# mjsargent/gym-miniworld

Measured on AMD Instinct MI355X. Metric: env-steps/s (80x60 RGB obs), higher is better.
Workload: dtype f64 sim / f32 render / u8 obs; 1 GPU; maze8192; env_id=MiniWorld-Maze-v0, envs_per_gpu=8192, global_envs=8192, obs=80x60 RGB, domain_rand=False, actions=uniform random over {turn_left, turn_right, move_forward}, counter-based, auto_reset=True, parallelism=env-sharded x1

## Files before the change

### gym_miniworld_amd/build.py

```python
import os
import subprocess
import sys

HERE = os.path.dirname(os.path.abspath(__file__))
CSRC = os.path.join(HERE, "csrc")
SOURCES = ["mwb_api.hip", "mwb_kernels.hip", "mwb_copy.hip", "mwb_repeat.hip", "mwb_rollout.hip"]
HEADERS = ["mwb_internal.h", "mwb_task_table.h", "mwb_copy_check.h", "mwb_repeat_fold.h", "mwb_rollout_map.h", "mwb_dispatch_map.h", "mwb_lds_layout.h", "mwb_glibc_trig.h", "mwb_sincos_table.inc", "mwb_texture_host.h", os.path.join("..", "..", "include", "miniworld_batch.h")]
OUT = os.path.join(HERE, "libmwbatch.so")
REMARKS = os.path.join(HERE, "libmwbatch.resources.txt")
FLAGS = ["--offload-arch=gfx950", "-O3", "-std=c++17", "-fPIC", "-shared", "-ffp-contract=off", "-Wall",
         "-Wno-unused-value"]


def needs_build():
    if not os.path.exists(OUT):
        return True
    t = os.path.getmtime(OUT)
    return any(os.path.getmtime(os.path.join(CSRC, f)) > t for f in SOURCES + HEADERS)


def source_digest():
    import hashlib
    h = hashlib.sha1()
    for f in SOURCES + HEADERS:
        with open(os.path.join(CSRC, f), "rb") as fh:
            h.update(fh.read())
    h.update(" ".join(FLAGS).encode())
    return h.hexdigest()


# ... 27 lines not shown
```

### gym_miniworld_amd/csrc/mwb_api.hip

```cpp
#include <math.h>
#include <stdio.h>
#include <stdlib.h>
#include <string.h>

#include <string>
#include <type_traits>
#include <vector>

#include "mwb_internal.h"
#include "mwb_lds_layout.h"
#include "mwb_rollout_map.h"
#include "mwb_task_table.h"
#include "mwb_texture_host.h"

static_assert(mwb_task_frame_words(1) == MWB_FRAME_WORDS_FOR(1) && mwb_task_frame_words(MWB_MAX_ENTS) == MWB_FRAME_WORDS_FOR(MWB_MAX_ENTS),
              "mwb_task_table.h restates the frame constants' size");

static thread_local std::string g_err;
static int set_err(int code, const std::string &msg) { g_err = msg; return code; }
#define HIP_TRY(expr)                                                                       \
    do {                                                                                    \
        hipError_t _e = (expr);                                                             \
        if (_e != hipSuccess)                                                               \
            return set_err(MWB_EHIP, std::string(#expr) + ": " + hipGetErrorString(_e));    \
// ... 200 lines not shown
    {
        std::string why;
        if (int rc = mwb_resolve_task(*cfg, &t, &why)) return set_err(rc, why);
    }

    mwb_handle *h = new mwb_handle();
    h->cfg = *cfg;
    h->serial = g_next_serial++;
    MwbDev &d = h->dev;
    d.N = cfg->num_envs; d.task = cfg->task; d.W = cfg->obs_width; d.H = cfg->obs_height;
    d.want_depth = cfg->want_depth ? 1 : 0; d.layout = cfg->layout; d.domain_rand = cfg->domain_rand ? 1 : 0;
    d.auto_reset = cfg->no_auto_reset ? 0 : 1;
    d.ent_task = t.ent_task; d.n_boxes = t.n_boxes; d.R_max = t.R_max; d.S_max = t.S_max; d.max_episode_steps = t.max_episode_steps;
    d.n_tex = t.n_tex; d.no_ceiling = t.no_ceiling; d.poly = t.poly; d.room_words = t.room_words; d.frame_words = t.frame_words;
    d.agent_radius = t.agent_radius;
    memcpy(d.task_args, t.task_args, sizeof(d.task_args));
    double P[MWB_NPARAM][9];
    if (cfg->use_default_params) default_params(P); else memcpy(P, cfg->params, sizeof(P));
    for (int i = 0; i < MWB_NPARAM; i++)
        for (int k = 0; k < 3; k++) { d.params[i].def[k] = P[i][k]; d.params[i].lo[k] = P[i][3 + k]; d.params[i].hi[k] = P[i][6 + k]; }
    d.stk_cpf = 3;
    { const char *dbg = getenv("MWB_DEBUG"); d.debug_flags = dbg ? atoi(dbg) : 0; }
    { const char *ex = getenv("MWB_EXP"); d.exp_flags = ex ? atoi(ex) : 0; }
    { const char *no = getenv("MWB_NO_OVERLAP"); h->overlap_reset = !(no && atoi(no)); }
    {
        const char *sp = getenv("MWB_SPLIT");
        int split = sp ? atoi(sp) : 768;
        d.split_envs = split < 0 ? 0 : (split > cfg->num_envs ? cfg->num_envs : split);
    }
    if (d.ent_task) {
        int tw_ = 0, th_ = 0;
        const char *tl = getenv("MWB_TILE");
        if (tl && sscanf(tl, "%dx%d", &tw_, &th_) != 2) { tw_ = 0; th_ = 0; }
        if (tw_ > 0 && th_ > 0) { d.tile_w = tw_ < d.W ? tw_ : d.W; d.tile_h = th_ < d.H ? th_ : d.H; }
    }
    if (d.tile_w == 0 && (mwb_render_lds_bytes(d) > 160 * 1024 || !mwb_pixel_queue_fits(d.W, d.H))) {
        int tw = 0, th = 0;
        mwb_view_tile(&tw, &th);
        d.tile_w = tw < d.W ? tw : d.W; d.tile_h = th < d.H ? th : d.H;
    }
    { const char *no = getenv("MWB_NO_FRAME_REUSE"); h->frame_reuse = !(no && atoi(no)) && d.tile_w == 0; }

    const size_t N = (size_t)d.N;
    int rc = MWB_OK;
    mwb_for_each_env_array(d, d, h->frame_reuse, [&](auto *&, auto *&p, const MwbEnvArray &a) {
        if (rc == MWB_OK) rc = dev_alloc(h, &p, mwb_env_array_elems(a, N));
// ... 728 lines not shown
    if (render) { rc = ensure_ready(dst); if (rc) return rc; }
    hipStream_t s = (hipStream_t)stream;
    MwbDev &d = dst->dev;
    if (!dst->copy_dst_pairs) { rc = dev_alloc(dst, &dst->copy_dst_pairs, (size_t)d.N); if (rc) return rc; }
    if (!dst->copy_src_mark) { rc = dev_alloc(dst, &dst->copy_src_mark, (size_t)d.N); if (rc) return rc; }
    if (!dst->copy_rejected) {
        rc = dev_alloc(dst, &dst->copy_rejected, (size_t)1); if (rc) return rc;
        HIP_TRY(hipDeviceSynchronize());
    }
    if (dst->copy_pairs_cap < (size_t)count) {
        if (dst->copy_pairs) { HIP_TRY(hipFree(dst->copy_pairs)); dst->copy_pairs = nullptr; dst->copy_pairs_cap = 0; }
        const size_t cap = (size_t)count < (size_t)d.N ? (size_t)d.N : (size_t)count;
        HIP_TRY(hipMalloc((void **)&dst->copy_pairs, cap * sizeof(int2)));
        dst->copy_pairs_cap = cap;
    }
    const int slot = copy_table_for(dst, src);
    if (slot < 0) return slot;
    const mwb_handle::CopyTable &tab = dst->copy_table[slot];
    mwb_launch_copy_validate(dst_idx_dev, src_idx_dev, count, d.N, src->dev.N, same ? 1 : 0, dst->copy_dst_pairs, dst->copy_src_mark,
                             dst->copy_pairs, dst->copy_rejected, s);
    rc = check_launch("copy_validate_kernel"); if (rc) return rc;
    mwb_launch_copy_envs(dst->copy_tables + (size_t)slot * MWB_COPY_TABLE_DESCS, tab.n_small, tab.small_chunks, tab.n_large, dst->copy_pairs, count, s);
    rc = check_launch("copy_envs_kernel"); if (rc) return rc;
    dst->have_world = true;
    if (render) {
        d.step_pass = 0; d.reuse_pass = 0;
        dst->timing_now = false;
        mwb_launch_copy_list(d, dst->copy_pairs, count, 0, s);
        rc = check_launch("copy_list_kernel"); if (rc) return rc;
        mwb_launch_prep(d, 1, s);
        rc = check_launch("prep_kernel"); if (rc) return rc;
        mwb_launch_render(d, 1, s);
        rc = check_launch("render_kernel"); if (rc) return rc;
        mwb_launch_copy_list(d, dst->copy_pairs, count, 1, s);
        rc = check_launch("copy_list_kernel"); if (rc) return rc;
    } else {
        mwb_launch_copy_list(d, dst->copy_pairs, count, 2, s);
        rc = check_launch("copy_list_kernel"); if (rc) return rc;
    }
    if (copy_window) {
        const size_t plane = (size_t)d.W * d.H * (dst->stack_dtype == 1 ? 4 : 1), C = (size_t)dst->stack_n * dst->stack_cpf;
        const size_t kd = dst->stack_planes ? (size_t)dst->stack_planes : C, ks = src->stack_planes ? (size_t)src->stack_planes : C;
        const size_t pd = dst->stack_planes ? (size_t)dst->stack_pos : 0, ps = src->stack_planes ? (size_t)src->stack_pos : 0;
        mwb_launch_copy_stack((char *)dst->stack, kd * plane, pd * plane, (const char *)src->stack, ks * plane, ps * plane, C * plane, dst->copy_pairs, count, s);
        rc = check_launch("copy_stack_kernel"); if (rc) return rc;
    }
// ... 390 lines not shown
```

### gym_miniworld_amd/csrc/mwb_copy.hip

```cpp
#include "mwb_internal.h"
#include "mwb_copy_check.h"

#define COPY_THREADS 256

__global__ void __launch_bounds__(COPY_THREADS) copy_validate_kernel(int phase, const int32_t *__restrict__ dst_idx, const int32_t *__restrict__ src_idx,
                                                                     int count, int n_dst, int n_src, int same_handle, int32_t *__restrict__ dst_pairs,
                                                                     uint8_t *__restrict__ src_mark, int2 *__restrict__ pairs,
                                                                     unsigned long long *__restrict__ rejected) {
    for (size_t i = (size_t)blockIdx.x * COPY_THREADS + threadIdx.x; i < (size_t)count; i += (size_t)gridDim.x * COPY_THREADS) {
        const int32_t dst = dst_idx[i], src = src_idx[i];
        if (phase == 0) {
            if (mwb_copy_counts_dst(dst, n_dst)) atomicAdd(dst_pairs + dst, 1);
            if (mwb_copy_marks_src(dst, src, n_src, same_handle)) src_mark[src] = 1;
        } else if (phase == 1) {
            const bool in = mwb_copy_index_ok(dst, n_dst);
            const int v = mwb_copy_verdict(dst, src, n_dst, n_src, same_handle, in ? dst_pairs[dst] : 0, in && same_handle ? src_mark[dst] : 0);
            pairs[i] = v == MWB_PAIR_COPY ? make_int2(dst, src) : make_int2(-1, -1);
            if (v == MWB_PAIR_REJECTED) atomicAdd(rejected, 1ull);
        } else {
            if (mwb_copy_counts_dst(dst, n_dst)) dst_pairs[dst] = 0;
            if (mwb_copy_marks_src(dst, src, n_src, same_handle)) src_mark[src] = 0;
        }
    }
}
// ... 34 lines not shown
            if (wide) for (uint32_t b = 0; b < t.elem; b += 8) *(uint64_t *)(d + b) = *(const uint64_t *)(s + b);
            else for (uint32_t b = 0; b < t.elem; b += 4) *(uint32_t *)(d + b) = *(const uint32_t *)(s + b);
        }
    }
}

__global__ void __launch_bounds__(COPY_THREADS) copy_list_kernel(MwbDev d, const int2 *__restrict__ pairs, int count, int what) {
    if (what == 1 && blockIdx.x == 0 && threadIdx.x == 0) d.reset_count[0] = 0;
    for (size_t i = (size_t)blockIdx.x * COPY_THREADS + threadIdx.x; i < (size_t)count; i += (size_t)gridDim.x * COPY_THREADS) {
        const int dst = pairs[i].x;
        if (dst < 0) continue;
        if (what == 0) {
            d.reset_set[dst] = 1;
            const int at = atomicAdd(d.reset_count, 1);
            if (at < d.N) d.reset_list[at] = dst;
        } else if (what == 1) {
            d.reset_set[dst] = 0;
        } else if (d.frame_cached) {
            d.frame_cached[dst] = 0;
        }
    }
}

#define COPY_STACK_RUN 32768
__global__ void __launch_bounds__(COPY_THREADS) copy_stack_kernel(char *dst, size_t env_bytes_dst, size_t off_dst, const char *src,
                                                                  size_t env_bytes_src, size_t off_src, size_t window_bytes, const int2 *__restrict__ pairs) {
    const int2 p = pairs[blockIdx.x];
    if (p.x < 0) return;
    const size_t b0 = (size_t)blockIdx.y * COPY_STACK_RUN, n = window_bytes - b0 < COPY_STACK_RUN ? window_bytes - b0 : COPY_STACK_RUN;
    copy_run(dst + (size_t)p.x * env_bytes_dst + off_dst + b0, src + (size_t)p.y * env_bytes_src + off_src + b0, n);
}

static inline unsigned pair_blocks(int count) {
    const long long b = ((long long)count + COPY_THREADS - 1) / COPY_THREADS;
    return (unsigned)(b < 1 ? 1 : b > 4096 ? 4096 : b);
}

void mwb_launch_copy_validate(const int32_t *dst_idx, const int32_t *src_idx, int count, int n_dst, int n_src, int same_handle,
                              int32_t *dst_pairs, uint8_t *src_mark, int2 *pairs, unsigned long long *rejected, hipStream_t s) {
    for (int phase = 0; phase < 3; phase++)
        hipLaunchKernelGGL(copy_validate_kernel, dim3(pair_blocks(count)), dim3(COPY_THREADS), 0, s, phase, dst_idx, src_idx, count, n_dst, n_src,
                           same_handle, dst_pairs, src_mark, pairs, rejected);
}

void mwb_launch_copy_envs(const MwbCopyDesc *table, int n_small, int small_chunks, int n_large, const int2 *pairs, int count, hipStream_t s) {
    if (n_small > 0 && small_chunks > 0)
        hipLaunchKernelGGL(copy_envs_kernel<false>, dim3((unsigned)small_chunks, pair_blocks(count)), dim3(COPY_THREADS), 0, s, table, n_small, pairs, count);
    if (n_large > 0)
        hipLaunchKernelGGL(copy_envs_kernel<true>, dim3((unsigned)count, (unsigned)n_large), dim3(COPY_THREADS), 0, s, table, n_small, pairs, count);
}

void mwb_launch_copy_list(const MwbDev &d, const int2 *pairs, int count, int what, hipStream_t s) {
    hipLaunchKernelGGL(copy_list_kernel, dim3(pair_blocks(count)), dim3(COPY_THREADS), 0, s, d, pairs, count, what);
}

void mwb_launch_copy_stack(char *dst, size_t env_bytes_dst, size_t off_dst, const char *src, size_t env_bytes_src, size_t off_src,
                           size_t window_bytes, const int2 *pairs, int count, hipStream_t s) {
    const unsigned runs = (unsigned)((window_bytes + COPY_STACK_RUN - 1) / COPY_STACK_RUN);
    hipLaunchKernelGGL(copy_stack_kernel, dim3((unsigned)count, runs), dim3(COPY_THREADS), 0, s, dst, env_bytes_dst, off_dst, src, env_bytes_src,
                       off_src, window_bytes, pairs);
}
```

### gym_miniworld_amd/csrc/mwb_internal.h

```cpp
#pragma once
#include <hip/hip_runtime.h>
#include <stdint.h>

#include "../../include/miniworld_batch.h"

#define MWB_MT_WORDS 625
#define MWB_MAX_TEX MWB_NUM_TEXTURES
#define MWB_MAX_LEVELS 12
#define MWB_MAX_BOXES 6
#define MWB_RESET_MAX_BLOCKS 4096
#define MWB_ENT_AGENT 255
#define MWB_ORDER_STRIDE 24

#define RW_MINX 0
#define RW_MAXX 1
#define RW_MINZ 2
#define RW_MAXZ 3
#define RW_HEIGHT 4
#define RW_TEX 5
#define RW_NBR01 6
#define RW_NBR23 7
#define RW_SIDE0 8
#define RW_SIDE_WORDS 4
#define RS_LO 0
#define RS_HI 1
#define RS_MAXY 2
#define RS_UORG 3
// ... 132 lines not shown
    int32_t *n_order;
    double *task_f;
    int32_t *task_i;
    int32_t *text_tex;
    int32_t *ovr_slot;
    double *ovr_pose;
    const MwbMeshDesc *mesh_desc;
    const float4 *mesh_data;
    MwbMeshDims mesh_dims[MWB_MAX_MESH_DIMS];
    int n_mesh_dims;
    uint8_t *frame_cache;
    float *depth_cache;
    uint8_t *frame_cached;
    uint8_t *frame_same;
    int reuse_pass;
    unsigned long long *reuse_stats;
    int tile_w, tile_h;
    unsigned long long *dbg_counters;
    int exp_flags;
    int32_t *render_list;
    int32_t *reuse_list;
    int32_t *list_counts;
    const uint8_t *frozen;
};

struct MwbEnvArray {
    const char *name;
    bool minor;
    uint32_t rows;
    size_t per;
    const char *not_copied;
};
static inline size_t mwb_env_array_elems(const MwbEnvArray &a, size_t N) { return N * a.rows * a.per; }

template <class Dev, class F>
static inline void mwb_for_each_env_array(Dev &s, Dev &d, bool frame_reuse, F &&f) {
#define MWB_MINOR(p, rows, per, when, why) if (when) f(s.p, d.p, MwbEnvArray{#p, true, (uint32_t)(rows), (size_t)(per), why})
#define MWB_MAJOR(p, count, when, why) if (when) f(s.p, d.p, MwbEnvArray{#p, false, 1u, (size_t)(count), why})
    const char *const COPIED = nullptr;
    const char *const OUTPUT = "an output of the last transition or render: the next one rewrites it";
    const char *const DISPATCH = "dispatch scratch: a heuristic or a work list rebuilt before every launch";
    const char *const CACHE = "the copy pass and the render it runs maintain the cached frames and their flags";
    const int B = s.n_boxes;
    const bool always = true, ent = s.ent_task != 0, depth = s.want_depth != 0;
    const size_t pixels = (size_t)s.W * s.H;
    MWB_MINOR(agent_x, 1, 1, always, COPIED); MWB_MINOR(agent_z, 1, 1, always, COPIED); MWB_MINOR(agent_dir, 1, 1, always, COPIED);
    MWB_MINOR(box_x, B, 1, always, COPIED); MWB_MINOR(box_z, B, 1, always, COPIED); MWB_MINOR(box_dir, B, 1, always, COPIED);
    MWB_MINOR(box_y, B, 1, always, COPIED); MWB_MINOR(box_color, B, 3, always, COPIED); MWB_MINOR(box_size, B, 1, always, COPIED);
    MWB_MINOR(carrying, 1, 1, always, COPIED); MWB_MINOR(goal_dist, 1, 1, always, COPIED);
    MWB_MINOR(episode_count, 1, 1, always, COPIED); MWB_MINOR(task_step_count, 1, 1, always, COPIED); MWB_MINOR(goal_idx, 1, 1, always, COPIED);
    MWB_MAJOR(cam, 4, always, COPIED); MWB_MAJOR(sky_color, 3, always, COPIED); MWB_MAJOR(light_pos, 3, always, COPIED);
    MWB_MAJOR(light_color, 3, always, COPIED); MWB_MAJOR(light_ambient, 3, always, COPIED);
    MWB_MINOR(step_count, 1, 1, always, COPIED); MWB_MINOR(n_rooms, 1, 1, always, COPIED); MWB_MINOR(n_segs, 1, 1, always, COPIED);
    MWB_MINOR(n_rrooms, 1, 1, always, COPIED);
    MWB_MAJOR(world_ext, 4, always, COPIED);
    MWB_MAJOR(rng, MWB_MT_WORDS, always, COPIED);
    MWB_MAJOR(rooms, (size_t)s.R_max * s.room_words, always, COPIED);
    MWB_MINOR(segs, s.S_max * 4, 1, always, COPIED);
    MWB_MINOR(ent_meta, B, 1, ent, COPIED); MWB_MINOR(ent_radius, B, 1, ent, COPIED); MWB_MINOR(ent_height, B, 1, ent, COPIED);
    MWB_MINOR(ent_scale, B, 1, ent, COPIED);
    MWB_MAJOR(ent_order, MWB_ORDER_STRIDE, ent, COPIED); MWB_MINOR(n_order, 1, 1, ent, COPIED);
    MWB_MINOR(task_f, 1, 1, ent, COPIED); MWB_MINOR(task_i, 1, 1, ent, COPIED); MWB_MAJOR(text_tex, 8, ent, COPIED);
    MWB_MINOR(ovr_slot, 1, 1, ent, COPIED); MWB_MAJOR(ovr_pose, 4, ent, COPIED);
    MWB_MAJOR(frame, s.frame_words, always, "prep_kernel rebuilds it before every render");
    MWB_MINOR(reset_set, 1, 1, always, "the copy pass sets and clears it around the render it runs");
    MWB_MINOR(reset_list, 1, 1, always, "the copy pass sets and clears it around the render it runs");
    MWB_MAJOR(obs, pixels * 3, always, OUTPUT); MWB_MAJOR(depth, pixels, depth, OUTPUT);
    MWB_MAJOR(cost, 2, always, DISPATCH); MWB_MINOR(bucket, 1, 1, always, DISPATCH);
    MWB_MINOR(order_bufs[0], 1, 1, always, DISPATCH); MWB_MINOR(order_bufs[1], 1, 1, always, DISPATCH);
    MWB_MINOR(render_list, 1, 1, always, DISPATCH); MWB_MINOR(reuse_list, 1, 1, always, DISPATCH);
    MWB_MAJOR(frame_cache, pixels * 3, frame_reuse, CACHE); MWB_MAJOR(depth_cache, pixels, frame_reuse && depth, CACHE);
    MWB_MINOR(frame_cached, 1, 1, frame_reuse, CACHE); MWB_MINOR(frame_same, 1, 1, frame_reuse, CACHE);
#undef MWB_MINOR
#undef MWB_MAJOR
}

struct MwbCopyDesc {
    const char *src;
    char *dst;
    uint32_t rows, elem;
    uint64_t src_stride, dst_stride;
    uint32_t first_chunk;
    uint32_t pad;
};
#define MWB_COPY_SMALL_ELEM 32
#define MWB_COPY_ROW_CHUNK 8

template <class F>
static inline void mwb_for_each_copied_array(const MwbDev &s, const MwbDev &d, F &&f) {
    mwb_for_each_env_array(s, d, false, [&](auto *sp, auto *dp, const MwbEnvArray &a) {
        if (a.not_copied) return;
        const uint64_t elem = sizeof(*sp) * a.per;
        f((const char *)sp, (char *)dp, a.rows, (uint32_t)elem, a.minor ? elem * (uint64_t)s.N : 0, a.minor ? elem * (uint64_t)d.N : 0);
    });
}

void mwb_launch_copy_validate(const int32_t *dst_idx, const int32_t *src_idx, int count, int n_dst, int n_src, int same_handle,
                              int32_t *dst_pairs, uint8_t *src_mark, int2 *pairs, unsigned long long *rejected, hipStream_t s);
void mwb_launch_copy_envs(const MwbCopyDesc *table, int n_small, int small_chunks, int n_large, const int2 *pairs, int count, hipStream_t s);
void mwb_launch_copy_list(const MwbDev &d, const int2 *pairs, int count, int what, hipStream_t s);
void mwb_launch_copy_stack(char *dst, size_t env_bytes_dst, size_t off_dst, const char *src, size_t env_bytes_src, size_t off_src,
                           size_t window_bytes, const int2 *pairs, int count, hipStream_t s);

void mwb_launch_repeat_fold(const MwbDev &d, int sub, int last, int repeat, const uint8_t *skip, const int32_t *counts, double *sum,
                            int32_t *taken, uint8_t *same, uint8_t *frozen, hipStream_t s);

struct MwbRollout {
    int N, T, nstack, R;
    int grey;
    int base, cursor;
    size_t frame_bytes;
    char *ring;
    uint8_t *age;
    float *reward, *mask, *feature;
    unsigned long long *rejected;
};
void mwb_launch_rollout_push(const MwbRollout &r, int t, int after_reset, const uint8_t *fresh_dev, const uint8_t *done, const float *reward,
                             const float *feature, hipStream_t s);
void mwb_launch_rollout_after_update(const MwbRollout &r, hipStream_t s);
void mwb_launch_rollout_gather(const MwbRollout &r, const int64_t *index, int count, void *out, int out_float, hipStream_t s);

void mwb_launch_step(const MwbDev &d, const int32_t *actions, const uint8_t *skip_mask, hipStream_t s);
void mwb_launch_clear_list(const MwbDev &d, hipStream_t s);
// ... 18 lines not shown
```

### gym_miniworld_amd/csrc/mwb_kernels.hip

```cpp
#include <type_traits>

#include "mwb_internal.h"
#include "mwb_glibc_trig.h"
#include "mwb_lds_layout.h"
#include "mwb_dispatch_map.h"

__device__ __forceinline__ double ref_sin(double x) { return mwb_trig::in_range(x) ? mwb_trig::sin_glibc(x) : sin(x); }
__device__ __forceinline__ double ref_cos(double x) { return mwb_trig::in_range(x) ? mwb_trig::cos_glibc(x) : cos(x); }

__device__ __forceinline__ uint32_t mt_temper(uint32_t y) {
    y ^= (y >> 11);
    y ^= (y << 7) & 0x9d2c5680u;
    y ^= (y << 15) & 0xefc60000u;
    y ^= (y >> 18);
    return y;
}

__device__ __forceinline__ uint32_t mt_mix(uint32_t a, uint32_t b, uint32_t c) {
    uint32_t y = (a & 0x80000000u) | (b & 0x7fffffffu);
    return c ^ (y >> 1) ^ ((y & 1u) ? 0x9908b0dfu : 0u);
}

struct MtSerial {
    uint32_t *key;
// ... 47 lines not shown
        uint32_t mask = rng;
        mask |= mask >> 1; mask |= mask >> 2; mask |= mask >> 4; mask |= mask >> 8; mask |= mask >> 16;
        uint32_t v;
        do { v = next32() & mask; } while (v > rng);
        return lo + (int)v;
    }
};

template <class SegPtr>
__device__ __forceinline__ bool seg_hit(SegPtr sg, double px, double pz, double radius) {
    double ax = sg[0], az = sg[1], bx = sg[2], bz = sg[3];
    double abx = bx - ax, abz = bz - az;
    double apx = px - ax, apz = pz - az;
    double dotAPAB = (apx * abx + 0.0) + apz * abz;
    double dotABAB = (abx * abx + 0.0) + abz * abz;
    double proj = dotAPAB / dotABAB;
    proj = proj < 0 ? 0 : (proj > 1 ? 1 : proj);
    double cx = ax + proj * abx, cz = az + proj * abz;
    double ddx = cx - px, ddz = cz - pz;
    double dist = sqrt((ddx * ddx + 0.0) + ddz * ddz);
    return dist < radius;
}


__device__ __forceinline__ double tagged_add(double a, bool a_f32, double b, bool b_f32, bool &res_f32) {
    res_f32 = a_f32 || b_f32;
    return res_f32 ? (double)((float)a + (float)b) : a + b;
}
__device__ __forceinline__ double tagged_add(double a, bool a_f32, double b, bool b_f32) { bool f; return tagged_add(a, a_f32, b, b_f32, f); }

__device__ __forceinline__ double box_radius(double size) {
    double sx = size, sz = size;
    return sqrt(sx * sx + sz * sz) / 2;
}

#define STEP_PARTS 8
template <int NBX>
__global__ void __launch_bounds__(64 * STEP_PARTS) step_kernel(MwbDev d, const int32_t *__restrict__ actions,
                                                                const uint8_t *__restrict__ skip) {
    __shared__ double s_nx[64], s_nz[64];
    __shared__ int s_move[64], s_hit[64];
    const int lane = threadIdx.x & 63, part = threadIdx.x >> 6;
    const int e = blockIdx.x * 64 + lane;
    const bool in_range = e < d.N;
    const bool frozen = in_range && d.frozen && d.frozen[e];
    const bool dummy = in_range && !frozen && skip && skip[e];
    const bool live = in_range && !dummy && !frozen;
    int sc = 0, a = -1;
    double ax = 0, az = 0, adir = 0, nx = 0, nz = 0, turn_step = 0;
    constexpr int NB = NBX;
    double bx[NBX], bz[NBX], by[NBX], brad[NBX], bsz[NBX];
#pragma unroll
    for (int b = 0; b < NBX; b++) { bx[b] = 0; bz[b] = 0; by[b] = 0; brad[b] = 0; bsz[b] = 0; }
    int carried = -1;
    bool same = true;
    const double arad = d.agent_radius;
    if (blockIdx.x == 0 && threadIdx.x == 0 && d.order_state[1]) {
        d.order_state[0] ^= 1; d.order_state[1] = 0;
    }
    if (part == 0) {
        s_move[lane] = 0; s_hit[lane] = 0;
        if (dummy) {
            d.reward[e] = -99.0f; d.reward64[e] = -99.0; d.done[e] = 0; d.ep_steps[e] = d.step_count[e];
            d.reset_set[e] = 0;
            d.feature[e * 2] = 0.0f; d.feature[e * 2 + 1] = 0.0f;
            if (d.frame_same) d.frame_same[e] = d.frame_cached[e];
        }
        if (live) {
            a = actions[(size_t)e * d.act_stride];
            if (d.act_stride == 2 && actions[(size_t)e * 2 + 1] != (a >> 31)) a = -1;
            ax = d.agent_x[e]; az = d.agent_z[e]; adir = d.agent_dir[e];
#pragma unroll
            for (int b = 0; b < NBX; b++)
                if (b < NB) {
                    const size_t be = (size_t)b * d.N + e;
                    bx[b] = d.box_x[be]; bz[b] = d.box_z[be]; by[b] = d.box_y[be]; bsz[b] = d.box_size[be]; brad[b] = box_radius(bsz[b]);
                }
            carried = d.carrying[e];
            MtSerial g;
            const bool use_rng = d.domain_rand || d.task == MWB_TASK_SIM2REAL_PUSH;
            if (use_rng) g.load(d.rng + (size_t)e * MWB_MT_WORDS);
// ... 32 lines not shown
                }
            }
            sc = d.step_count[e] + 1;
            d.step_count[e] = sc;
            double fwd_step = d.params[MWB_P_FORWARD_STEP].def[0];
            double fwd_drift = d.params[MWB_P_FORWARD_DRIFT].def[0];
            turn_step = d.params[MWB_P_TURN_STEP].def[0];
            if (d.domain_rand) {
                fwd_step = g.uniform(d.params[MWB_P_FORWARD_STEP].lo[0], d.params[MWB_P_FORWARD_STEP].hi[0]);
                fwd_drift = g.uniform(d.params[MWB_P_FORWARD_DRIFT].lo[0], d.params[MWB_P_FORWARD_DRIFT].hi[0]);
                turn_step = g.uniform(d.params[MWB_P_TURN_STEP].lo[0], d.params[MWB_P_TURN_STEP].hi[0]);
            }
            if (use_rng) g.store();
            if (a == 2 || a == 3) {
                double fd = (a == 2) ? fwd_step : -fwd_step;
                double c = ref_cos(adir), s = ref_sin(adir);
                nx = (ax + c * fd) + s * fwd_drift;
                nz = (az + (-s) * fd) + c * fwd_drift;
                s_nx[lane] = nx; s_nz[lane] = nz; s_move[lane] = 1;
            }
        }
    }
    __syncthreads();
    if (live && s_move[lane]) {
        const double px = s_nx[lane], pz = s_nz[lane];
        const double *sg = d.segs + e;
        const size_t N = (size_t)d.N;
        const int ns = d.n_segs[e];
        bool hit = false;
        const double guard = arad + 1e-9;
        for (int i0 = part * 8; i0 < ns; i0 += 8 * STEP_PARTS) {
            double q[8][4];
#pragma unroll
            for (int k = 0; k < 8; k++) {
                const int i = (i0 + k < ns) ? i0 + k : ns - 1;
#pragma unroll
                for (int c = 0; c < 4; c++) q[k][c] = sg[(size_t)(i * 4 + c) * N];
            }
#pragma unroll
            for (int k = 0; k < 8; k++) {
                bool nearby = px >= fmin(q[k][0], q[k][2]) - guard && px <= fmax(q[k][0], q[k][2]) + guard &&
                              pz >= fmin(q[k][1], q[k][3]) - guard && pz <= fmax(q[k][1], q[k][3]) + guard;
                if (nearby) hit = seg_hit(q[k], px, pz, arad) || hit;
            }
        }
        if (hit) s_hit[lane] = 1;
    }
    __syncthreads();
    if (part != 0 || !live) return;
    const double max_fwd = d.params[MWB_P_FORWARD_STEP].hi[0];
    auto pick = [&](const double (&v)[NBX], int i) {
        double r_ = v[0];
#pragma unroll
        for (int b = 1; b < NBX; b++) r_ = (i == b) ? v[b] : r_;
        return r_;
    };
    auto intersect_serial = [&](int self_idx, double px, double pz, double radius, bool test_walls) {
        if (test_walls) {
            const int ns = d.n_segs[e];
            for (int i = 0; i < ns; i++) {
                double q[4];
#pragma unroll
                for (int c = 0; c < 4; c++) q[c] = d.segs[(size_t)(i * 4 + c) * d.N + e];
                if (seg_hit(q, px, pz, radius)) return 1;
            }
        }
        int res = 0;
#pragma unroll
        for (int b = NBX - 1; b >= 0; b--) {
            const double ddx = bx[b] - px, ddz = bz[b] - pz;
            const bool h = b < NB && b != self_idx && sqrt(ddx * ddx + 0.0 + ddz * ddz) < radius + brad[b];
            res = h ? 2 + b : res;
        }
        if (!res && self_idx != NB) {
            const double ddx = ax - px, ddz = az - pz;
            if (sqrt(ddx * ddx + 0.0 + ddz * ddz) < radius + arad) res = 2 + NB;
        }
        return res;
    };
    auto carry_pos = [&](double agx, double agz, double dir, double &cx, double &cy, double &cz) {
        const double er = pick(brad, carried);
        const double dist = (arad + er) + max_fwd;
        const double c = ref_cos(dir), s_ = ref_sin(dir);
        cx = agx + (c * 1.05) * dist; cz = agz + ((-s_) * 1.05) * dist;
        const double eh = pick(bsz, carried);
        double yp = (d.cam[e * 4 + 0] - eh) - 0.3;
        yp = yp > 0 ? yp : 0;
        cy = (0.0 + (0.0 * 1.05) * dist) + 1.0 * yp;
        cx = cx + 0.0 * yp; cz = cz + 0.0 * yp;
// ... 112 lines not shown
    int a = actions[(size_t)e * d.act_stride];
    if (d.act_stride == 2 && actions[(size_t)e * 2 + 1] != (a >> 31)) a = -1;
    double ax = d.agent_x[e], az = d.agent_z[e], adir = d.agent_dir[e];
    const double arad = d.agent_radius;
    uint8_t *ord = d.ent_order + (size_t)e * MWB_ORDER_STRIDE;
    int n_ord = d.n_order[e];
    int carried = d.carrying[e];
    const double max_fwd = d.params[MWB_P_FORWARD_STEP].hi[0];
    const double cam_height = d.cam[e * 4 + 0];
    const int ns = d.n_segs[e];
    bool same = carried < 0 && d.ovr_slot[e] < 0;
    d.ovr_slot[e] = -1;
    MtSerial g;
    const bool use_rng = d.domain_rand || d.task == MWB_TASK_COLLECTHEALTH;
    if (use_rng) g.load(d.rng + (size_t)e * MWB_MT_WORDS);
    const int sc = d.step_count[e] + 1;
    d.step_count[e] = sc;
    double fwd_step = d.params[MWB_P_FORWARD_STEP].def[0], fwd_drift = d.params[MWB_P_FORWARD_DRIFT].def[0], turn_step = d.params[MWB_P_TURN_STEP].def[0];
    if (d.domain_rand) {
        fwd_step = g.uniform(d.params[MWB_P_FORWARD_STEP].lo[0], d.params[MWB_P_FORWARD_STEP].hi[0]);
        fwd_drift = g.uniform(d.params[MWB_P_FORWARD_DRIFT].lo[0], d.params[MWB_P_FORWARD_DRIFT].hi[0]);
        turn_step = g.uniform(d.params[MWB_P_TURN_STEP].lo[0], d.params[MWB_P_TURN_STEP].hi[0]);
    }
    auto walls_hit = [&](double px, double pz, double radius) {
        for (int i = 0; i < ns; i++) {
            double q[4];
#pragma unroll
            for (int c = 0; c < 4; c++) q[c] = d.segs[(size_t)(i * 4 + c) * N + e];
            if (seg_hit(q, px, pz, radius)) return true;
        }
        return false;
    };
    auto intersect = [&](int self_slot, double px, double pz, double radius, bool rf32) {
        if (walls_hit(px, pz, radius)) return 1;
        for (int k = 0; k < n_ord; k++) {
            const int slot = ord[k];
            if (slot == self_slot) continue;
            double ox, oz, orad; bool of32 = false;
            if (slot == MWB_ENT_AGENT) { ox = ax; oz = az; orad = arad; }
            else { const size_t be = (size_t)slot * N + e; ox = d.box_x[be]; oz = d.box_z[be]; orad = d.ent_radius[be]; of32 = MWB_META_RADF32(d.ent_meta[be]) != 0; }
            const double ddx = ox - px, ddz = oz - pz;
            if (sqrt(ddx * ddx + 0.0 + ddz * ddz) < tagged_add(radius, rf32, orad, of32)) return 2 + (slot == MWB_ENT_AGENT ? E : slot);
        }
        return 0;
    };
    auto carry_pos = [&](int slot, double agx, double agz, double dir, double &cx, double &cy, double &cz) {
        const size_t be = (size_t)slot * N + e;
        bool f32;
        double dist = tagged_add(arad, false, d.ent_radius[be], MWB_META_RADF32(d.ent_meta[be]) != 0, f32);
        dist = tagged_add(dist, f32, max_fwd, false);
        const double c = ref_cos(dir), s_ = ref_sin(dir);
        cx = agx + (c * 1.05) * dist; cz = agz + ((-s_) * 1.05) * dist;
        double yp = (cam_height - d.ent_height[be]) - 0.3;
        yp = yp > 0 ? yp : 0;
        cy = (0.0 + (0.0 * 1.05) * dist) + 1.0 * yp;
// ... 998 lines not shown
        }
        for (int k = 0; k < 3; k++) {
            d.sky_color[e * 3 + k] = sky[k]; d.light_pos[e * 3 + k] = lpos[k];
            d.light_color[e * 3 + k] = lcol[k]; d.light_ambient[e * 3 + k] = lamb[k];
        }
        d.carrying[e] = -1;
        d.goal_idx[e] = goal_idx; d.episode_count[e] = episode_count;
        d.goal_dist[e] = goal_dist;
        for (int k = 0; k < 4; k++) d.cam[e * 4 + k] = cam[k];
        d.step_count[e] = 0;
        d.n_rooms[e] = w.fail ? -1 : w.n_rooms;
        {
            double mnx = rooms[0].min_x, mxx = rooms[0].max_x, mnz = rooms[0].min_z, mxz = rooms[0].max_z;
            for (int i = 1; i < w.n_rooms; i++) {
                mnx = fmin(mnx, rooms[i].min_x); mxx = fmax(mxx, rooms[i].max_x);
                mnz = fmin(mnz, rooms[i].min_z); mxz = fmax(mxz, rooms[i].max_z);
            }
            d.world_ext[e * 4 + 0] = mnx; d.world_ext[e * 4 + 1] = mxx; d.world_ext[e * 4 + 2] = mnz; d.world_ext[e * 4 + 3] = mxz;
        }
        if (w.fail) atomicExch(d.error_flag, e + 1);
        d.n_segs[e] = w.n_segs;
    }
    for (int i = lane; i < w.n_segs * 4; i += WAVE) d.segs[(size_t)i * d.N + e] = segs[i];
    float *grooms = d.rooms + (size_t)e * d.R_max * d.room_words;
    auto culled = [&](const LRoom &r) {
        double cx = 0, cz = 0, inward = 0;
        for (int k = 0; k < r.ne; k++) { cx += r.ox[k] / r.ne; cz += r.oz[k] / r.ne; }
        for (int k = 0; k < r.ne; k++) {
            double nx, nz;
            w.edge_normal(r, k, nx, nz);
            inward += nx * (cx - r.ox[k]) + nz * (cz - r.oz[k]);
        }
        return inward < 0;
    };
    for (int ri = lane; d.poly && ri < w.n_rooms; ri += WAVE) {
        const LRoom &r = rooms[ri];
        float *o = grooms + (size_t)ri * MWB_POLY_ROOM_WORDS;
        const bool cull_r = culled(r);
        o[PW_HEIGHT] = d.no_ceiling ? -(float)r.height : (float)r.height;
        o[PW_TEX] = __int_as_float(r.tex_id[0] | (r.tex_id[1] << 8) | (r.tex_id[2] << 16));
        o[PW_FLAGS] = __int_as_float(r.ne | (cull_r ? 256 : 0));
        o[3] = 0.0f;
        for (int k = 0; k < 4; k++) {
            float *ed = o + PW_EDGE0 + PW_EDGE_WORDS * k;
            for (int q = 0; q < PW_EDGE_WORDS; q++) ed[q] = 0.0f;
            ed[9] = __int_as_float(-1);
// ... 2125 lines not shown
}

void mwb_launch_stack(const MwbDev &d, void *stack, int nstack, int dtype, int after_reset, hipStream_t s, int cpf) {
    const int plane4 = (d.W * d.H) / 4;
    dim3 grid((plane4 + 255) / 256, d.N);
    if (dtype == 1) stack_kernel<float4, true><<<grid, dim3(256), 0, s>>>(d, (float4 *)stack, nstack * cpf, cpf, after_reset);
    else stack_kernel<uint32_t, false><<<grid, dim3(256), 0, s>>>(d, (uint32_t *)stack, nstack * cpf, cpf, after_reset);
}

#define GREY_CONVERT_RUN 4096
__global__ void __launch_bounds__(256) grey_convert_kernel(const uint8_t *__restrict__ rgb, float *__restrict__ grey, int runs_per_frame, int plane, int cwh, int vec) {
    const int f = blockIdx.x / runs_per_frame, run = blockIdx.x - f * runs_per_frame;
    const int p0 = run * GREY_CONVERT_RUN, p1 = plane - p0 < GREY_CONVERT_RUN ? plane : p0 + GREY_CONVERT_RUN;
    grey_put_range<256>(rgb + (size_t)f * plane * 3, grey + (size_t)f * plane, nullptr, cwh, plane, p0, p1, vec);
}
void mwb_launch_grey_convert(const uint8_t *rgb, float *grey, int n_frames, int plane, int layout, hipStream_t s) {
    const int runs = (plane + GREY_CONVERT_RUN - 1) / GREY_CONVERT_RUN;
    const int vec = plane % 4 == 0 && ((uintptr_t)rgb & 3) == 0 && ((uintptr_t)grey & 15) == 0;
    grey_convert_kernel<<<dim3((unsigned)n_frames * (unsigned)runs), dim3(256), 0, s>>>(rgb, grey, runs, plane, layout == MWB_LAYOUT_CWH, vec);
}

__global__ void intersect_kernel(MwbDev d, int e, int ent, double x, double z, double radius, int *result) {
    if (threadIdx.x != 0 || blockIdx.x != 0) return;
    int ns = d.n_segs[e], res = 0;
    for (int i = 0; i < ns && !res; i++) {
        double q[4];
        for (int c = 0; c < 4; c++) q[c] = d.segs[(size_t)(i * 4 + c) * d.N + e];
        if (seg_hit(q, x, z, radius)) res = 1;
    }
    if (d.ent_task) {
        const uint8_t *ord = d.ent_order + (size_t)e * MWB_ORDER_STRIDE;
        const int n_ord = d.n_order[e];
        for (int k = 0; k < n_ord && !res; k++) {
            const int slot = ord[k];
            if (slot == (ent == d.n_boxes ? MWB_ENT_AGENT : ent)) continue;
            double ox, oz, orad; bool of32 = false;
            if (slot == MWB_ENT_AGENT) { ox = d.agent_x[e]; oz = d.agent_z[e]; orad = d.agent_radius; }
            else { const size_t be = (size_t)slot * d.N + e; ox = d.box_x[be]; oz = d.box_z[be]; orad = d.ent_radius[be]; of32 = MWB_META_RADF32(d.ent_meta[be]) != 0; }
            const double ddx = ox - x, ddz = oz - z;
            if (sqrt(ddx * ddx + 0.0 + ddz * ddz) < tagged_add(radius, false, orad, of32)) res = 2 + (slot == MWB_ENT_AGENT ? d.n_boxes : slot);
        }
        *result = res;
        return;
    }
    for (int b = 0; b < d.n_boxes && !res; b++) {
        if (b == ent) continue;
        double ddx = d.box_x[(size_t)b * d.N + e] - x, ddz = d.box_z[(size_t)b * d.N + e] - z;
        if (sqrt(ddx * ddx + 0.0 + ddz * ddz) < radius + box_radius(d.box_size[(size_t)b * d.N + e])) res = 2 + b;
    }
    if (!res && ent != d.n_boxes) {
        double ddx = d.agent_x[e] - x, ddz = d.agent_z[e] - z;
        if (sqrt(ddx * ddx + 0.0 + ddz * ddz) < radius + d.agent_radius) res = 2 + d.n_boxes;
// ... 581 lines not shown
```

Measured before the change: 14.65 million env-steps/s.

## Cull wall collision tests with per-group segment bounding boxes

Adds conservative f32 bounding boxes for each group of eight wall segments, built at reset and rebuilt after env copies. The step kernel skips segment groups whose box cannot reach the agent and redistributes surviving groups across the eight parts per env. For large segment counts it also reads a row-major copy of the segments. The aim is to cut the double-precision seg_hit work and strided segment loads in mazes with many walls. The cost is extra memory, extra writes at reset and copy, and more syncthreads in the step kernel.

```diff
diff --git a/gym_miniworld_amd/build.py b/gym_miniworld_amd/build.py
--- a/gym_miniworld_amd/build.py
+++ b/gym_miniworld_amd/build.py
@@ -5,7 +5,7 @@
 HERE = os.path.dirname(os.path.abspath(__file__))
 CSRC = os.path.join(HERE, "csrc")
 SOURCES = ["mwb_api.hip", "mwb_kernels.hip", "mwb_copy.hip", "mwb_repeat.hip", "mwb_rollout.hip"]
-HEADERS = ["mwb_internal.h", "mwb_task_table.h", "mwb_copy_check.h", "mwb_repeat_fold.h", "mwb_rollout_map.h", "mwb_dispatch_map.h", "mwb_lds_layout.h", "mwb_glibc_trig.h", "mwb_sincos_table.inc", "mwb_texture_host.h", os.path.join("..", "..", "include", "miniworld_batch.h")]
+HEADERS = ["mwb_internal.h", "mwb_task_table.h", "mwb_copy_check.h", "mwb_repeat_fold.h", "mwb_rollout_map.h", "mwb_dispatch_map.h", "mwb_seg_groups.h", "mwb_lds_layout.h", "mwb_glibc_trig.h", "mwb_sincos_table.inc", "mwb_texture_host.h", os.path.join("..", "..", "include", "miniworld_batch.h")]
 OUT = os.path.join(HERE, "libmwbatch.so")
 REMARKS = os.path.join(HERE, "libmwbatch.resources.txt")
 FLAGS = ["--offload-arch=gfx950", "-O3", "-std=c++17", "-fPIC", "-shared", "-ffp-contract=off", "-Wall",
diff --git a/gym_miniworld_amd/csrc/mwb_api.hip b/gym_miniworld_amd/csrc/mwb_api.hip
--- a/gym_miniworld_amd/csrc/mwb_api.hip
+++ b/gym_miniworld_amd/csrc/mwb_api.hip
@@ -246,6 +246,7 @@
     d.stk_cpf = 3;
     { const char *dbg = getenv("MWB_DEBUG"); d.debug_flags = dbg ? atoi(dbg) : 0; }
     { const char *ex = getenv("MWB_EXP"); d.exp_flags = ex ? atoi(ex) : 0; }
+    { const char *no = getenv("MWB_NO_SEG_CULL"); d.no_seg_cull = no && atoi(no); }
     { const char *no = getenv("MWB_NO_OVERLAP"); h->overlap_reset = !(no && atoi(no)); }
     {
         const char *sp = getenv("MWB_SPLIT");
@@ -1020,6 +1021,8 @@
     rc = check_launch("copy_validate_kernel"); if (rc) return rc;
     mwb_launch_copy_envs(dst->copy_tables + (size_t)slot * MWB_COPY_TABLE_DESCS, tab.n_small, tab.small_chunks, tab.n_large, dst->copy_pairs, count, s);
     rc = check_launch("copy_envs_kernel"); if (rc) return rc;
+    mwb_launch_copy_seg_box(d, dst->copy_pairs, count, s);
+    rc = check_launch("copy_seg_box_kernel"); if (rc) return rc;
     dst->have_world = true;
     if (render) {
         d.step_pass = 0; d.reuse_pass = 0;
diff --git a/gym_miniworld_amd/csrc/mwb_copy.hip b/gym_miniworld_amd/csrc/mwb_copy.hip
--- a/gym_miniworld_amd/csrc/mwb_copy.hip
+++ b/gym_miniworld_amd/csrc/mwb_copy.hip
@@ -1,5 +1,6 @@
 #include "mwb_internal.h"
 #include "mwb_copy_check.h"
+#include "mwb_seg_groups.h"
 
 #define COPY_THREADS 256
 
@@ -80,6 +81,27 @@
     }
 }
 
+__global__ void __launch_bounds__(COPY_THREADS) copy_seg_box_kernel(MwbDev d, const int2 *__restrict__ pairs, int count) {
+    const size_t G = (size_t)mwb_seg_groups(d.S_max), N = (size_t)d.N;
+    for (size_t i = (size_t)blockIdx.x * COPY_THREADS + threadIdx.x; i < (size_t)count * G; i += (size_t)gridDim.x * COPY_THREADS) {
+        const int dst = pairs[i / G].x, g = (int)(i % G);
+        if (dst < 0) continue;
+        const int ns = d.n_segs[dst] < d.S_max ? d.n_segs[dst] : d.S_max, n = ns - g * MWB_SEG_GROUP < MWB_SEG_GROUP ? ns - g * MWB_SEG_GROUP : MWB_SEG_GROUP;
+        if (n < 1) continue;
+        double q[MWB_SEG_GROUP * 4];
+#pragma unroll
+        for (int k = 0; k < MWB_SEG_GROUP * 4; k++) q[k] = d.segs[((size_t)g * MWB_SEG_GROUP * 4 + (k < n * 4 ? k : 0)) * N + dst];
+        const MwbSegBox b = mwb_seg_group_box(q, n);
+        float *o = d.seg_box + (size_t)g * 4 * N + dst;
+        o[0] = b.min_x; o[N] = b.min_z; o[2 * N] = b.max_x; o[3 * N] = b.max_z;
+        if (d.seg_rows) {
+            double *r = d.seg_rows + ((size_t)dst * d.S_max + (size_t)g * MWB_SEG_GROUP) * 4;
+#pragma unroll
+            for (int k = 0; k < MWB_SEG_GROUP * 4; k++) if (k < n * 4) r[k] = q[k];
+        }
+    }
+}
+
 #define COPY_STACK_RUN 32768
 __global__ void __launch_bounds__(COPY_THREADS) copy_stack_kernel(char *dst, size_t env_bytes_dst, size_t off_dst, const char *src,
                                                                   size_t env_bytes_src, size_t off_src, size_t window_bytes, const int2 *__restrict__ pairs) {
@@ -112,6 +134,11 @@
     hipLaunchKernelGGL(copy_list_kernel, dim3(pair_blocks(count)), dim3(COPY_THREADS), 0, s, d, pairs, count, what);
 }
 
+void mwb_launch_copy_seg_box(const MwbDev &d, const int2 *pairs, int count, hipStream_t s) {
+    const long long b = ((long long)count * mwb_seg_groups(d.S_max) + COPY_THREADS - 1) / COPY_THREADS;
+    hipLaunchKernelGGL(copy_seg_box_kernel, dim3((unsigned)(b < 1 ? 1 : b > 4096 ? 4096 : b)), dim3(COPY_THREADS), 0, s, d, pairs, count);
+}
+
 void mwb_launch_copy_stack(char *dst, size_t env_bytes_dst, size_t off_dst, const char *src, size_t env_bytes_src, size_t off_src,
                            size_t window_bytes, const int2 *pairs, int count, hipStream_t s) {
     const unsigned runs = (unsigned)((window_bytes + COPY_STACK_RUN - 1) / COPY_STACK_RUN);
diff --git a/gym_miniworld_amd/csrc/mwb_internal.h b/gym_miniworld_amd/csrc/mwb_internal.h
--- a/gym_miniworld_amd/csrc/mwb_internal.h
+++ b/gym_miniworld_amd/csrc/mwb_internal.h
@@ -3,6 +3,7 @@
 #include <stdint.h>
 
 #include "../../include/miniworld_batch.h"
+#include "mwb_seg_groups.h"
 
 #define MWB_MT_WORDS 625
 #define MWB_MAX_TEX MWB_NUM_TEXTURES
@@ -181,7 +182,11 @@
     int32_t *reuse_list;
     int32_t *list_counts;
     const uint8_t *frozen;
-};
+    float *seg_box;
+    int no_seg_cull;
+    double *seg_rows;
+};
+MWB_SEG_HD static inline bool mwb_step_culls(int S_max) { return mwb_seg_groups(S_max) > 8; }
 
 struct MwbEnvArray {
     const char *name;
@@ -216,6 +221,8 @@
     MWB_MAJOR(rng, MWB_MT_WORDS, always, COPIED);
     MWB_MAJOR(rooms, (size_t)s.R_max * s.room_words, always, COPIED);
     MWB_MINOR(segs, s.S_max * 4, 1, always, COPIED);
+    MWB_MINOR(seg_box, mwb_seg_groups(s.S_max) * 4, 1, always, "derived from segs: copy_seg_box_kernel rebuilds it from the copied segments");
+    MWB_MAJOR(seg_rows, (size_t)s.S_max * 4, mwb_step_culls(s.S_max), "derived from segs: copy_seg_box_kernel rebuilds it from the copied segments");
     MWB_MINOR(ent_meta, B, 1, ent, COPIED); MWB_MINOR(ent_radius, B, 1, ent, COPIED); MWB_MINOR(ent_height, B, 1, ent, COPIED);
     MWB_MINOR(ent_scale, B, 1, ent, COPIED);
     MWB_MAJOR(ent_order, MWB_ORDER_STRIDE, ent, COPIED); MWB_MINOR(n_order, 1, 1, ent, COPIED);
@@ -258,6 +265,7 @@
                               int32_t *dst_pairs, uint8_t *src_mark, int2 *pairs, unsigned long long *rejected, hipStream_t s);
 void mwb_launch_copy_envs(const MwbCopyDesc *table, int n_small, int small_chunks, int n_large, const int2 *pairs, int count, hipStream_t s);
 void mwb_launch_copy_list(const MwbDev &d, const int2 *pairs, int count, int what, hipStream_t s);
+void mwb_launch_copy_seg_box(const MwbDev &d, const int2 *pairs, int count, hipStream_t s);
 void mwb_launch_copy_stack(char *dst, size_t env_bytes_dst, size_t off_dst, const char *src, size_t env_bytes_src, size_t off_src,
                            size_t window_bytes, const int2 *pairs, int count, hipStream_t s);
 
diff --git a/gym_miniworld_amd/csrc/mwb_kernels.hip b/gym_miniworld_amd/csrc/mwb_kernels.hip
--- a/gym_miniworld_amd/csrc/mwb_kernels.hip
+++ b/gym_miniworld_amd/csrc/mwb_kernels.hip
@@ -93,6 +93,23 @@
     return dist < radius;
 }
 
+__device__ __forceinline__ bool walls_hit_serial(const MwbDev &d, int e, int ns, double px, double pz, double radius) {
+    const size_t N = (size_t)d.N;
+    const double guard = radius + 1e-9;
+    for (int g = 0; g * MWB_SEG_GROUP < ns; g++) {
+        const float *b = d.seg_box + (size_t)g * 4 * N + e;
+        if (!d.no_seg_cull && !mwb_seg_box_near(b[0], b[N], b[2 * N], b[3 * N], px, pz, guard)) continue;
+        const int i1 = (g + 1) * MWB_SEG_GROUP < ns ? (g + 1) * MWB_SEG_GROUP : ns;
+        for (int i = g * MWB_SEG_GROUP; i < i1; i++) {
+            double q[4];
+#pragma unroll
+            for (int c = 0; c < 4; c++) q[c] = d.segs[(size_t)(i * 4 + c) * N + e];
+            if (seg_hit(q, px, pz, radius)) return true;
+        }
+    }
+    return false;
+}
+
 
 __device__ __forceinline__ double tagged_add(double a, bool a_f32, double b, bool b_f32, bool &res_f32) {
     res_f32 = a_f32 || b_f32;
@@ -106,11 +123,13 @@
 }
 
 #define STEP_PARTS 8
+#define STEP_BOXES 4
 template <int NBX>
 __global__ void __launch_bounds__(64 * STEP_PARTS) step_kernel(MwbDev d, const int32_t *__restrict__ actions,
                                                                 const uint8_t *__restrict__ skip) {
     __shared__ double s_nx[64], s_nz[64];
     __shared__ int s_move[64], s_hit[64];
+    __shared__ uint8_t s_near[STEP_PARTS][64];
     const int lane = threadIdx.x & 63, part = threadIdx.x >> 6;
     const int e = blockIdx.x * 64 + lane;
     const bool in_range = e < d.N;
@@ -128,6 +147,17 @@
     const double arad = d.agent_radius;
     if (blockIdx.x == 0 && threadIdx.x == 0 && d.order_state[1]) {
         d.order_state[0] ^= 1; d.order_state[1] = 0;
+    }
+    const size_t segN = (size_t)d.N;
+    const int NG = mwb_seg_groups(d.S_max);
+    static_assert(STEP_PARTS == 8, "mwb_step_culls (mwb_internal.h) states the same threshold");
+    const bool cull = mwb_step_culls(d.S_max);
+    float bb[STEP_BOXES][4];
+#pragma unroll
+    for (int j = 0; j < STEP_BOXES; j++) {
+        const int g = part + j * STEP_PARTS < NG ? part + j * STEP_PARTS : 0;
+#pragma unroll
+        for (int c = 0; c < 4; c++) bb[j][c] = cull && in_range ? d.seg_box[(size_t)(g * 4 + c) * segN + e] : 0.0f;
     }
     if (part == 0) {
         s_move[lane] = 0; s_hit[lane] = 0;
@@ -206,20 +236,22 @@
         }
     }
     __syncthreads();
-    if (live && s_move[lane]) {
+    {
+        const bool mover = live && s_move[lane];
         const double px = s_nx[lane], pz = s_nz[lane];
         const double *sg = d.segs + e;
-        const size_t N = (size_t)d.N;
-        const int ns = d.n_segs[e];
+        const int ns = mover ? d.n_segs[e] : 0, ng = mwb_seg_groups(ns);
         bool hit = false;
         const double guard = arad + 1e-9;
-        for (int i0 = part * 8; i0 < ns; i0 += 8 * STEP_PARTS) {
+        const double *qb = cull ? d.seg_rows + (size_t)e * d.S_max * 4 : sg;
+        const size_t qs = cull ? 1 : segN;
+        auto test_batch = [&](int i0) {
             double q[8][4];
 #pragma unroll
             for (int k = 0; k < 8; k++) {
                 const int i = (i0 + k < ns) ? i0 + k : ns - 1;
 #pragma unroll
-                for (int c = 0; c < 4; c++) q[k][c] = sg[(size_t)(i * 4 + c) * N];
+                for (int c = 0; c < 4; c++) q[k][c] = qb[(size_t)(i * 4 + c) * qs];
             }
 #pragma unroll
             for (int k = 0; k < 8; k++) {
@@ -227,6 +259,37 @@
                               pz >= fmin(q[k][1], q[k][3]) - guard && pz <= fmax(q[k][1], q[k][3]) + guard;
                 if (nearby) hit = seg_hit(q[k], px, pz, arad) || hit;
             }
+        };
+        if (!cull) {
+            for (int i0 = part * MWB_SEG_GROUP; i0 < ns; i0 += MWB_SEG_GROUP * STEP_PARTS) test_batch(i0);
+        }
+        for (int c0 = 0; cull && c0 < NG; c0 += STEP_PARTS * STEP_BOXES) {
+            if (c0 > 0) {
+#pragma unroll
+                for (int j = 0; j < STEP_BOXES; j++) {
+                    const int g = c0 + part + j * STEP_PARTS < NG ? c0 + part + j * STEP_PARTS : 0;
+#pragma unroll
+                    for (int c = 0; c < 4; c++) bb[j][c] = mover ? d.seg_box[(size_t)(g * 4 + c) * segN + e] : 0.0f;
+                }
+            }
+            unsigned near = 0;
+#pragma unroll
+            for (int j = 0; j < STEP_BOXES; j++)
+                if (c0 + part + j * STEP_PARTS < ng && (d.no_seg_cull || mwb_seg_box_near(bb[j][0], bb[j][1], bb[j][2], bb[j][3], px, pz, guard))) near |= 1u << j;
+            s_near[part][lane] = (uint8_t)near;
+            __syncthreads();
+            unsigned todo = 0;
+            if (mover) {
+#pragma unroll
+                for (int p = 0; p < STEP_PARTS; p++) todo |= (unsigned)s_near[p][lane] << (p * STEP_BOXES);
+            }
+            for (int k = 0; k < part && todo; k++) todo &= todo - 1;
+            while (todo) {
+                const int b = __ffs(todo) - 1;
+                for (int k = 0; k < STEP_PARTS && todo; k++) todo &= todo - 1;
+                test_batch((c0 + b / STEP_BOXES + (b % STEP_BOXES) * STEP_PARTS) * MWB_SEG_GROUP);
+            }
+            if (c0 + STEP_PARTS * STEP_BOXES < NG) __syncthreads();
         }
         if (hit) s_hit[lane] = 1;
     }
@@ -240,15 +303,7 @@
         return r_;
     };
     auto intersect_serial = [&](int self_idx, double px, double pz, double radius, bool test_walls) {
-        if (test_walls) {
-            const int ns = d.n_segs[e];
-            for (int i = 0; i < ns; i++) {
-                double q[4];
-#pragma unroll
-                for (int c = 0; c < 4; c++) q[c] = d.segs[(size_t)(i * 4 + c) * d.N + e];
-                if (seg_hit(q, px, pz, radius)) return 1;
-            }
-        }
+        if (test_walls && walls_hit_serial(d, e, d.n_segs[e], px, pz, radius)) return 1;
         int res = 0;
 #pragma unroll
         for (int b = NBX - 1; b >= 0; b--) {
@@ -407,15 +462,7 @@
         fwd_drift = g.uniform(d.params[MWB_P_FORWARD_DRIFT].lo[0], d.params[MWB_P_FORWARD_DRIFT].hi[0]);
         turn_step = g.uniform(d.params[MWB_P_TURN_STEP].lo[0], d.params[MWB_P_TURN_STEP].hi[0]);
     }
-    auto walls_hit = [&](double px, double pz, double radius) {
-        for (int i = 0; i < ns; i++) {
-            double q[4];
-#pragma unroll
-            for (int c = 0; c < 4; c++) q[c] = d.segs[(size_t)(i * 4 + c) * N + e];
-            if (seg_hit(q, px, pz, radius)) return true;
-        }
-        return false;
-    };
+    auto walls_hit = [&](double px, double pz, double radius) { return walls_hit_serial(d, e, ns, px, pz, radius); };
     auto intersect = [&](int self_slot, double px, double pz, double radius, bool rf32) {
         if (walls_hit(px, pz, radius)) return 1;
         for (int k = 0; k < n_ord; k++) {
@@ -1460,6 +1507,13 @@
         d.n_segs[e] = w.n_segs;
     }
     for (int i = lane; i < w.n_segs * 4; i += WAVE) d.segs[(size_t)i * d.N + e] = segs[i];
+    if (d.seg_rows) for (int i = lane; i < w.n_segs * 4; i += WAVE) d.seg_rows[(size_t)e * d.S_max * 4 + i] = segs[i];
+    for (int g = lane; g < mwb_seg_groups(w.n_segs); g += WAVE) {
+        const int n = w.n_segs - g * MWB_SEG_GROUP;
+        const MwbSegBox b = mwb_seg_group_box(segs + g * MWB_SEG_GROUP * 4, n < MWB_SEG_GROUP ? n : MWB_SEG_GROUP);
+        float *o = d.seg_box + (size_t)g * 4 * d.N + e;
+        o[0] = b.min_x; o[(size_t)d.N] = b.min_z; o[2 * (size_t)d.N] = b.max_x; o[3 * (size_t)d.N] = b.max_z;
+    }
     float *grooms = d.rooms + (size_t)e * d.R_max * d.room_words;
     auto culled = [&](const LRoom &r) {
         double cx = 0, cz = 0, inward = 0;
@@ -3631,12 +3685,7 @@
 
 __global__ void intersect_kernel(MwbDev d, int e, int ent, double x, double z, double radius, int *result) {
     if (threadIdx.x != 0 || blockIdx.x != 0) return;
-    int ns = d.n_segs[e], res = 0;
-    for (int i = 0; i < ns && !res; i++) {
-        double q[4];
-        for (int c = 0; c < 4; c++) q[c] = d.segs[(size_t)(i * 4 + c) * d.N + e];
-        if (seg_hit(q, x, z, radius)) res = 1;
-    }
+    int res = walls_hit_serial(d, e, d.n_segs[e], x, z, radius) ? 1 : 0;
     if (d.ent_task) {
         const uint8_t *ord = d.ent_order + (size_t)e * MWB_ORDER_STRIDE;
         const int n_ord = d.n_order[e];
diff --git a/gym_miniworld_amd/csrc/mwb_seg_groups.h b/gym_miniworld_amd/csrc/mwb_seg_groups.h
--- /dev/null
+++ b/gym_miniworld_amd/csrc/mwb_seg_groups.h
@@ -0,0 +1,50 @@
+#pragma once
+#include <math.h>
+#include <stdint.h>
+
+#if defined(__HIPCC__) || defined(__CUDACC__)
+#define MWB_SEG_HD __host__ __device__
+#define MWB_SEG_UNROLL _Pragma("unroll")
+#else
+#define MWB_SEG_HD
+#define MWB_SEG_UNROLL
+#endif
+
+#define MWB_SEG_GROUP 8
+
+struct MwbSegBox { float min_x, min_z, max_x, max_z; };
+
+MWB_SEG_HD static inline int mwb_seg_groups(int n_segs) { return (n_segs + MWB_SEG_GROUP - 1) / MWB_SEG_GROUP; }
+
+MWB_SEG_HD static inline float mwb_f32_below(double v) {
+    float f = (float)v;
+    if ((double)f > v) f = nextafterf(f, -INFINITY);
+    return (double)f <= v ? f : -INFINITY;
+}
+MWB_SEG_HD static inline float mwb_f32_above(double v) {
+    float f = (float)v;
+    if ((double)f < v) f = nextafterf(f, INFINITY);
+    return (double)f >= v ? f : INFINITY;
+}
+
+MWB_SEG_HD static inline MwbSegBox mwb_seg_group_box(const double *segs, int n) {
+    const MwbSegBox all = {-INFINITY, -INFINITY, INFINITY, INFINITY};
+    if (n < 1) return all;
+    if (n > MWB_SEG_GROUP) n = MWB_SEG_GROUP;
+    double mnx = INFINITY, mnz = INFINITY, mxx = -INFINITY, mxz = -INFINITY;
+    MWB_SEG_UNROLL
+    for (int i = 0; i < MWB_SEG_GROUP; i++) {
+        if (i >= n) break;
+        const double ax = segs[i * 4 + 0], az = segs[i * 4 + 1], bx = segs[i * 4 + 2], bz = segs[i * 4 + 3];
+        if (!(fabs(ax) <= 1.7976931348623157e308 && fabs(az) <= 1.7976931348623157e308 &&
+              fabs(bx) <= 1.7976931348623157e308 && fabs(bz) <= 1.7976931348623157e308)) return all;
+        mnx = ax < mnx ? ax : mnx; mnx = bx < mnx ? bx : mnx; mxx = ax > mxx ? ax : mxx; mxx = bx > mxx ? bx : mxx;
+        mnz = az < mnz ? az : mnz; mnz = bz < mnz ? bz : mnz; mxz = az > mxz ? az : mxz; mxz = bz > mxz ? bz : mxz;
+    }
+    const MwbSegBox b = {mwb_f32_below(mnx), mwb_f32_below(mnz), mwb_f32_above(mxx), mwb_f32_above(mxz)};
+    return b;
+}
+
+MWB_SEG_HD static inline bool mwb_seg_box_near(float min_x, float min_z, float max_x, float max_z, double px, double pz, double guard) {
+    return px >= (double)min_x - guard && px <= (double)max_x + guard && pz >= (double)min_z - guard && pz <= (double)max_z + guard;
+}
```

New measurement: 14.90 million env-steps/s (median of 6 runs). 1.02x the previous value.
